# cbalint13/opencv-dlco

Hardware: AMD Instinct MI355X
Metric: pj-learn patch-pairs/sec (higher is better)
Workload: dtype f32; 1 GPU; pj-learn configs[1] Liberty-shaped, rank ~64: 500000 pair-rows x PR-dim 8192, batch 200+200 per GPU (global 200+200), mu=0.0025 gamma=0.5, fp32, rank 48 after 3893 steps; device= (gfx950:sramecc+:xnack-), burn_in_steps=300

## Files before the change

### include/dlco.h

```cpp
#ifndef DLCO_H
#define DLCO_H

#include <stddef.h>
#include <stdint.h>

#ifdef __cplusplus
extern "C" {
#endif

#define DLCO_OK            0
#define DLCO_ERR_INVALID  -2
#define DLCO_ERR_HIP      -3
#define DLCO_ERR_NODEVICE -4
#define DLCO_ERR_NOCONV   -5
#define DLCO_ERR_COMM     -6

typedef struct dlco_ctx dlco_ctx;

typedef struct dlco_cfg {
    int32_t  F;
    int32_t  N;
    int32_t  B;
    float    mu;
    float    gamma;
// ... 86 lines not shown
    int32_t        rows, ld;
    int32_t        kmajor;
    const int32_t *row_ids, *row_ids2;
    const float   *row_scale;
} dlco_gemm_operand;
typedef struct dlco_gemm_probe_args {
    int32_t M, N, K;
    dlco_gemm_operand A, B;
    const float *B2_host;
    int32_t split_k, k_dev, small_m_tiles, small_n_tiles, depth, reps;
    float   alpha, beta, b1, b2;
    const float *E1_host, *E2_host;
} dlco_gemm_probe_args;
int dlco_gemm_probe(dlco_ctx *ctx, const dlco_gemm_probe_args *args, float *C_host, float *C2_host, int32_t *depth_used,
                    double *us_per_launch);
int dlco_hinge_sum(dlco_ctx *ctx, const float *pos_host, int32_t n_pos,
                   const float *neg_host, int32_t n_neg, double *out);
int dlco_roc_stats(dlco_ctx *ctx, const float *dist_host, const uint8_t *labels_host, int32_t n,
                   float *fpr95, double *auc);

typedef struct dlco_log_entry {
    uint32_t t;
    int32_t  is_best;
    int32_t  saved;
    float    loss_val, regul, obj, obj_best;
    int32_t  rank, rank_best;
    int32_t  dim;
    double   auc, auc_best;
    float    fpr95, fpr95_best;
    double   vtime;
// ... 131 lines not shown
```

### opencv-dlco_amd/__init__.py

```python
import ctypes as C
import os
import subprocess

import numpy as np

_HERE = os.path.dirname(os.path.abspath(__file__))
LIB_PATH = os.path.join(_HERE, "libdlco.so")
HEADER_PATH = os.path.join(os.path.dirname(_HERE), "include", "dlco.h")

OK, ERR_INVALID, ERR_HIP, ERR_NODEVICE, ERR_NOCONV, ERR_COMM = 0, -2, -3, -4, -5, -6
BUF_DIST, BUF_GRAD, BUF_DFAVG, BUF_W, BUF_GATHER, BUF_DATA = 1, 2, 3, 4, 5, 6
ALLGATHER_FN = C.CFUNCTYPE(C.c_int, C.c_void_p, C.c_int32, C.c_size_t)
DETECT_THRESHOLD = 100 * 100 * 256 * 256


class DlcoError(RuntimeError):
    def __init__(self, code, msg):
        super().__init__("libdlco error %d: %s" % (code, msg))
        self.code = code


class Cfg(C.Structure):
    _fields_ = [
        ("F", C.c_int32), ("N", C.c_int32), ("B", C.c_int32),
# ... 22 lines not shown
    _fields_ = [
        ("host", C.POINTER(C.c_float)), ("rows", C.c_int32), ("ld", C.c_int32), ("kmajor", C.c_int32),
        ("row_ids", C.POINTER(C.c_int32)), ("row_ids2", C.POINTER(C.c_int32)), ("row_scale", C.POINTER(C.c_float)),
    ]


class GemmProbeArgs(C.Structure):
    _fields_ = [
        ("M", C.c_int32), ("N", C.c_int32), ("K", C.c_int32),
        ("A", GemmOperand), ("B", GemmOperand),
        ("B2_host", C.POINTER(C.c_float)),
        ("split_k", C.c_int32), ("k_dev", C.c_int32), ("small_m_tiles", C.c_int32), ("small_n_tiles", C.c_int32),
        ("depth", C.c_int32), ("reps", C.c_int32),
        ("alpha", C.c_float), ("beta", C.c_float), ("b1", C.c_float), ("b2", C.c_float),
        ("E1_host", C.POINTER(C.c_float)), ("E2_host", C.POINTER(C.c_float)),
    ]


def build(verbose=False):
    cmd = ["make", "-C", os.path.join(_HERE, "csrc"), "-j8"]
    if not verbose:
        cmd.insert(1, "-s")
    subprocess.check_call(cmd)


_lib = None
f32p, i32p, u8p = C.POINTER(C.c_float), C.POINTER(C.c_int32), C.POINTER(C.c_uint8)


def load():
# ... 34 lines not shown
    L.dlco_get_batch.argtypes = [vp, i32p, i32p, f32p, f32p, i32p, i32p]
    L.dlco_get_t.argtypes = [vp, C.POINTER(C.c_uint32)]
    L.dlco_get_W.argtypes = [vp, f32p, i32p]
    L.dlco_get_A.argtypes = [vp, f32p]
    L.dlco_get_dfavg.argtypes = [vp, f32p]
    L.dlco_set_state.argtypes = [vp, C.c_uint32, f32p, f32p, C.c_int32]
    L.dlco_validate.argtypes = [vp, f32p, f32p, i32p]
    L.dlco_stats.argtypes = [vp, f32p, C.c_int32, i32p, f32p, C.POINTER(C.c_double)]
    L.dlco_project_sqdist.argtypes = [vp, i32p, C.c_int32, f32p, C.c_int32, f32p]
    L.dlco_viol_counts.argtypes = [vp, f32p, f32p, C.c_int32, i32p, i32p]
    L.dlco_grad_rda.argtypes = [vp, i32p, i32p, i32p, i32p, C.c_int32, C.c_float, C.c_float, f32p, f32p]
    L.dlco_psd_project.argtypes = [vp, f32p, C.c_uint32, f32p, i32p, f32p]
    L.dlco_hinge_sum.argtypes = [vp, f32p, C.c_int32, f32p, C.c_int32, C.POINTER(C.c_double)]
    L.dlco_sym_product.argtypes = [vp, f32p, C.c_int32, f32p, C.c_int32, f32p]
    L.dlco_gemm_probe.argtypes = [vp, C.POINTER(GemmProbeArgs), f32p, f32p, i32p, C.POINTER(C.c_double)]
    L.dlco_roc_stats.argtypes = [vp, f32p, u8p, C.c_int32, f32p, C.POINTER(C.c_double)]
    L.dlco_log_step.argtypes = [vp, C.POINTER(LogEntry)]
    L.dlco_get_saved.argtypes = [vp, f32p, i32p, f32p]
    L.dlco_profile_enable.argtypes = [vp, C.c_int32]
    L.dlco_profile_read.argtypes = [vp, C.c_char_p, C.POINTER(C.c_int64), C.POINTER(C.c_double)]
    L.dlco_eig_stats.argtypes = [vp, C.POINTER(C.c_int64), C.POINTER(C.c_int64), C.POINTER(C.c_int64), i32p]
    L.dlco_counters.argtypes = [vp, C.POINTER(C.c_int64)]
    i64 = C.c_int64
    L.dlco_set_pairs_device.argtypes = [vp, vp, C.c_int32, i32p]
    L.dlco_desc_last_error.restype = C.c_char_p
    L.dlco_desc_last_error.argtypes = [vp]
    L.dlco_desc_create.argtypes = [C.POINTER(vp), C.c_float, C.c_int32, C.c_int32, C.c_int32]
    L.dlco_desc_destroy.argtypes = [vp]
    L.dlco_desc_destroy.restype = None
    L.dlco_desc_select_filters.argtypes = [f32p, C.c_int32, C.c_int32, f32p, C.c_int32, f32p, C.POINTER(C.c_int32)]
# ... 352 lines not shown
        twin = None if B2 is None else _f32(B2)
        assert twin is None or twin.shape == b.shape
        e1, e2 = (None if e is None else _f32(e) for e in (E1, E2))
        assert all(e is None or e.shape == (M, N) for e in (e1, e2))
        a.B2_host, a.E1_host, a.E2_host = _p(twin, f32p), _p(e1, f32p), _p(e2, f32p)
        a.split_k, a.k_dev, a.depth, a.reps = split_k, k_dev, depth, reps
        a.small_m_tiles, a.small_n_tiles = int(small_m_tiles), int(small_n_tiles)
        a.alpha, a.beta, a.b1, a.b2 = alpha, beta, b1, b2
        out = np.zeros((M, N), np.float32) if C_in is None else np.array(C_in, dtype=np.float32, order="C")
        assert out.shape == (M, N)
        out2 = None if twin is None else out.copy()
        used, us = C.c_int32(), C.c_double()
        self._ck(self.L.dlco_gemm_probe(self.h, C.byref(a), _p(out, f32p), _p(out2, f32p), C.byref(used), C.byref(us)))
        return dict(C=out, C2=out2, depth=used.value, us=us.value if reps else None)

    def hinge_sum(self, pos, neg):
        p, n = _f32(pos), _f32(neg)
        out = C.c_double()
        self._ck(self.L.dlco_hinge_sum(self.h, _p(p, f32p), p.size, _p(n, f32p), n.size, C.byref(out)))
        return out.value

    def roc_stats(self, dist, labels):
        d, l = _f32(dist), np.ascontiguousarray(labels, np.uint8).ravel()
        f, a = C.c_float(), C.c_double()
        self._ck(self.L.dlco_roc_stats(self.h, _p(d, f32p), _p(l, u8p), d.size, C.byref(f), C.byref(a)))
        return f.value, a.value

    def profile_enable(self, on=True):
        self._ck(self.L.dlco_profile_enable(self.h, int(on)))

# ... 485 lines not shown
```

### opencv-dlco_amd/csrc/dlco_api.cpp

```cpp
#include "../../include/dlco.h"

#include "dlco_internal.hpp"
#include "eig_tracker.hpp"
#include "pair_index.hpp"
#include "rccl_comm.hpp"
#include "host_comm.hpp"

#include <algorithm>
#include <cfloat>
#include <chrono>
#include <cmath>
#include <cstring>

using namespace dlco;

static thread_local std::string g_last_error;

namespace {
struct EnvSwitch { const char *name, *purpose; };
const EnvSwitch kEnvSwitches[] = {
    {"DLCO_SYRK_FP32", "gradient SYRK as the k-ordered fp32 MFMA chain (syrk_rda_kernel8) instead of split-bf16 planes"},
    {"DLCO_NO_PACKED", "full F x F dual average where the packed upper-tile form would apply"},
    {"DLCO_FORCE_SHARD", "column-sharded layout (cfg.shard) on a single rank: the multi-GPU path on one GPU"},
    {"DLCO_NO_RANK_UPDATE", "first filter term from a product with the dual average, not from the step's rank update"},
// ... 43 lines not shown
    int32_t *pin_ids = nullptr;
    uint32_t upload_ctr = 0;
    struct IdView { int32_t *p = nullptr; };
    DevBuf<int32_t> ids_all;
    IdView pos_rows, neg_rows, local_ids;
    const float *pd_cur = nullptr, *nd_cur = nullptr;
    DevBuf<int32_t> rho, kappa, act_ids, seed_ids, act_slot;
    bool rank_update = false;
    int planes_mode = 0;
    const float *ru_proj = nullptr;
    int ru_rows = 0;
    DevBuf<float> act_w, seed_w, dist_x, pd, nd, proj_slab, vproj, vdist, hrows;
    DevBuf<char> pplane[3];
    float *xdist = nullptr, *xgrad = nullptr;
    DevBuf<int> k_active;
    DevBuf<double> dscal;
    size_t proj_slab_floats = 0;
    int phase = 0;
    EigTracker *eig = nullptr;
    DevBuf<char> syrk_planes;
    RocWork *roc = nullptr;
    int64_t nonconv_steps = 0, steps_run = 0, active_rows_sum = 0;
    int32_t nonconv_window = 0;

    double auc_best = 0.0;
    float obj_best = FLT_MAX, fpr95_best = FLT_MAX;
    int r_best = 0;
    DevBuf<float> W_save_dev;
    int r_save = 0;
    int r_save_dev = 0;
// ... 145 lines not shown
    c->vproj.alloc((size_t)r * VCHUNK);
    for (int c0 = 0; c0 < n; c0 += VCHUNK) {
        const int nc = std::min(VCHUNK, n - c0);
        GemmArgs g;
        g.M = r; g.N = nc; g.K = c->F;
        g.A.p = Wd; g.A.ld = c->F; g.A.kmajor = false;
        g.B.ld = c->F; g.B.kmajor = false;
        if (rr.a) { g.B.p = c->dists; g.B.row_ids = rr.a + c0; g.B.row_ids2 = rr.b ? rr.b + c0 : nullptr; }
        else g.B.p = c->dists + (size_t)(row0 + c0) * c->F;
        g.C = c->vproj.p; g.ldc = VCHUNK;
        gemm_f32(g, c->stream);
        sqdist_from_proj(c->vproj.p, 1, r, nc, VCHUNK, out_dev + c0, c->stream);
    }
}

void project_few(dlco_ctx *c, const int32_t *ids_dev, int n, const float *Wd, int r, float *out_dev, int r_ext = 0)
{
    c->ru_proj = nullptr; c->ru_rows = 0;
    if (n <= 0) return;
    if (r <= 0) { fill_f32(out_dev, 0.f, (size_t)n, c->stream); return; }
    const int rp = std::max(r, r_ext);
    if (c->cfg.grad_bf16 && rp <= 96) {
        const int blocks = (n + 127) / 128;
        int ks = 1;
        while (ks * 2 * blocks <= 256 && (c->F / 64) % (ks * 2) == 0) ks *= 2;
        const size_t need = (size_t)(ks + 1) * rp * n;
        if (need > c->proj_slab_floats) { sync(c); c->proj_slab.alloc(need); c->proj_slab_floats = need; }
        float *reduced = rp > r ? c->proj_slab.p + (size_t)ks * rp * n : nullptr;
        for (auto &pl : c->pplane) pl.alloc(project_rows_plane_bytes(c->F));
        const RowRef rr = rows_of(c, ids_dev, 0, n);
        c->prof.begin(PROF_PROJECT);
// ... 19 lines not shown
    const int bn = (n <= 64 || bm == 64) ? 64 : 128;
    const long tiles = (long)((rp + bm - 1) / bm) * ((n + bn - 1) / bn);
    const int split = split_k_slices(tiles, 512, c->F, 128, LONG_MAX);
    const size_t need = (size_t)(split + 1) * rp * n;
    if (need > c->proj_slab_floats) { sync(c); c->proj_slab.alloc(need); c->proj_slab_floats = need; }
    float *proj = c->proj_slab.p + (size_t)split * rp * n;
    GemmArgs g;
    g.M = rp; g.N = n; g.K = c->F;
    g.A.p = Wd; g.A.ld = c->F; g.A.kmajor = false;
    const RowRef rr = rows_of(c, ids_dev, 0, n);
    g.B.p = c->dists; g.B.ld = c->F; g.B.kmajor = false; g.B.row_ids = rr.a; g.B.row_ids2 = rr.b;
    g.C = proj; g.ldc = n;
    g.split_k = split; g.slab = c->proj_slab.p;
    g.small_m_tiles = bm == 64;
    g.small_n_tiles = bn == 64;
    c->prof.begin(PROF_PROJECT);
    gemm_f32(g, c->stream);
    sqdist_from_proj(proj, 1, r, n, n, out_dev, c->stream);
    c->prof.end(PROF_PROJECT);
    if (rp > r) { c->ru_proj = proj; c->ru_rows = rp; }
}

void grad_syrk(dlco_ctx *c, const int32_t *ids, const float *w, const int *k_dev, int kmax, float alpha, float beta,
               float *dst, bool packed = false, const RankCoeffJob *coeff_job = nullptr)
{
    const int kpad = (kmax + 31) & ~31;
    const RowRef rr = rows_of(c, ids, 0, kpad);
    if (c->F % 128 == 0 && (reinterpret_cast<uintptr_t>(c->dists) & 15) == 0 &&
        (!c->shard || (c->comm.c0 % 128 == 0 && c->comm.cw % 128 == 0))) {
        c->prof.begin(PROF_GRAD_SYRK);
        const size_t pbytes = syrk_planes_bytes(kpad, c->F);
        if (pbytes > c->syrk_planes.n) { sync(c); c->syrk_planes.alloc(pbytes); }
        SyrkArgs a;
// ... 50 lines not shown
    const int B = c->B, Bl = c->Bl;
    for (int k = 0; k < B; k++) {
        const int ip = c->rng.uniform(0, c->idx.n_pos_trn);
        const int in = c->rng.uniform(0, c->idx.n_neg_trn);
        c->h_pos_rows[k] = c->idx.pos[ip];
        c->h_neg_rows[k] = c->idx.neg[in];
    }
    const size_t n_ids = (size_t)2 * B + 2 * Bl;
    int32_t *slot = c->pin_ids + (size_t)(c->upload_ctr++ & 1u) * n_ids;
    std::memcpy(slot, c->h_pos_rows.data(), B * sizeof(int32_t));
    std::memcpy(slot + B, c->h_neg_rows.data(), B * sizeof(int32_t));
    std::memcpy(slot + 2 * B, c->h_pos_rows.data() + c->lo, Bl * sizeof(int32_t));
    std::memcpy(slot + 2 * B + Bl, c->h_neg_rows.data() + c->lo, Bl * sizeof(int32_t));
    DLCO_HIP(hipMemcpyAsync(c->ids_all.p, slot, n_ids * sizeof(int32_t), hipMemcpyHostToDevice, c->stream));
    const int r_ext = (c->rank_update && c->r > 0 && c->eig->ext_rows() > c->r) ? c->eig->ext_rows() : 0;
    project_few(c, c->local_ids.p, 2 * Bl, c->W.p, c->r, c->xdist + (size_t)c->cfg.rank * 2 * Bl, r_ext);
    c->phase = 1;
}

void step_grad(dlco_ctx *c)
{
    DLCO_CHECK(c->phase == 1, DLCO_ERR_INVALID, "dlco_step_grad: call dlco_step_begin first");
    DLCO_CHECK(!c->shard, DLCO_ERR_INVALID, "dlco_step_grad: a sharded context steps with dlco_step");
    const int B = c->B, Bl = c->Bl, world = c->cfg.world;
    gather_dists(c, &c->pd_cur, &c->nd_cur);
    viol_counts_active_rows(c->pd_cur, c->nd_cur, B, c->rho.p, c->kappa.p, c->pos_rows.p, c->neg_rows.p, c->lo, c->lo + Bl,
                            c->act_ids.p, c->act_w.p, c->k_active.p, c->act_slot.p, c->stream);
    float alpha, beta;
    rda_coeffs(c, &alpha, &beta);
    RankCoeffJob job;
    const bool have_job = c->rank_update && c->planes_mode == 3 && c->ru_proj && world == 1 && c->eig->rank_coeff_job(&job, (2 * Bl + 31) & ~31);
    if (have_job) { job.proj = c->ru_proj; job.ldp = 2 * Bl; job.slot = c->act_slot.p; }
    if (world == 1) grad_syrk(c, c->act_ids.p, c->act_w.p, c->k_active.p, 2 * Bl, alpha, beta, c->dfavg.p, c->packed, have_job ? &job : nullptr);
    else grad_syrk(c, c->act_ids.p, c->act_w.p, c->k_active.p, 2 * Bl, 1.0f, 0.0f, c->xgrad);
    if (c->rank_update && c->ru_proj && c->syrk_planes.p) {
        RankUpdate ru;
        ru.proj = c->ru_proj; ru.ldp = 2 * Bl; ru.rows = c->ru_rows;
        ru.slot = c->act_slot.p; ru.w = c->act_w.p; ru.k_dev = c->k_active.p; ru.kmax = (2 * Bl + 31) & ~31;
        ru.planes = c->syrk_planes.p; ru.alpha = alpha; ru.beta = beta;
        ru.coeff_ready = have_job && job.m == c->ru_rows;
        ru.planes_mode = c->planes_mode;
        c->eig->offer_rank_update(ru);
// ... 156 lines not shown
        const int B = c->B;
        c->h_pos_rows.assign(B, 0); c->h_neg_rows.assign(B, 0);
        DLCO_HIP(hipHostMalloc((void **)&c->pin_ids, (size_t)2 * (2 * B + 2 * c->Bl) * sizeof(int32_t)));
        c->ids_all.alloc((size_t)2 * B + 2 * c->Bl);
        c->pos_rows.p = c->ids_all.p; c->neg_rows.p = c->ids_all.p + B; c->local_ids.p = c->ids_all.p + 2 * B;
        c->rho.alloc(B); c->kappa.alloc(B);
        const int kcap = (2 * B + 31) & ~31;
        c->act_ids.alloc(kcap); c->act_w.alloc(kcap); c->seed_ids.alloc(kcap); c->seed_w.alloc(kcap); c->act_slot.alloc(kcap);
        c->planes_mode = syrk_planes_mode(cfg->grad_bf16 != 0);
        c->rank_update = c->packed && cfg->world == 1 && c->planes_mode != 0 && env_switch("DLCO_NO_RANK_UPDATE") == nullptr;
        c->eig->set_emit_guards(c->rank_update);
        c->dist_x.alloc(2 * B); c->pd.alloc(B); c->nd.alloc(B);
        c->xdist = c->dist_x.p; c->xgrad = c->grad.p;
        c->k_active.alloc(4);
        c->k_active.zero(c->stream);
        c->eig->set_readback_extra(c->k_active.p);
        if (c->cfg.world == 1 || c->shard) {
            c->eig->set_growth_rows([c](float *dst, int want) -> int {
                if (c->phase != 2 || !c->have_data) return 0;
                const int k = c->eig->readback_extra();
                if (k <= 0 || k > 2 * c->B) return 0;
                const int cnt = std::min(want, k);
                if (cnt <= 0) return 0;
                const RowRef rr = rows_of(c, c->act_ids.p + (k - cnt), 0, cnt);
                scale_rows(dst, c->F, c->dists, c->F, nullptr, rr.a, rr.b, cnt, c->F, c->stream);
                return cnt;
            });
        }
        c->dscal.alloc(4);
        if (c->shard) {
// ... 648 lines not shown
            float ms = 0.f;
            DLCO_HIP(hipEventElapsedTime(&ms, e0, e1));
            (void)hipEventDestroy(e0); (void)hipEventDestroy(e1);
            if (us_per_launch) *us_per_launch = 1e3 * ms / a->reps;
        }
        h2d(c, C.p, C_host, mn * sizeof(float));
        if (C2_host) h2d(c, C2.p, C2_host, mn * sizeof(float));
        gemm_f32(g, c->stream);
        sync(c);
        d2h(c, C_host, C.p, mn * sizeof(float));
        if (C2_host) d2h(c, C2_host, C2.p, mn * sizeof(float));
        if (depth_used) *depth_used = used;
    });
}

int dlco_hinge_sum(dlco_ctx *c, const float *pos_host, int32_t n_pos, const float *neg_host, int32_t n_neg, double *out)
{
    if (!c || !out || n_pos < 0 || n_neg < 0) return DLCO_ERR_INVALID;
    return guarded(c, [&] {
        DLCO_HIP(hipSetDevice(c->cfg.device));
        *out = 0.0;
        if (n_pos == 0) return;
        DevBuf<float> p, n, rows;
        p.alloc(n_pos); n.alloc(std::max(n_neg, 1)); rows.alloc(n_pos);
        h2d(c, p.p, pos_host, (size_t)n_pos * sizeof(float));
        if (n_neg) h2d(c, n.p, neg_host, (size_t)n_neg * sizeof(float));
        hinge_rows(p.p, n_pos, n.p, n_neg, rows.p, c->stream);
        sum_f32_to_f64(rows.p, n_pos, c->dscal.p, c->stream);
        d2h(c, out, c->dscal.p, sizeof(double));
    });
// ... 128 lines not shown
```

### opencv-dlco_amd/csrc/dlco_internal.hpp

```cpp
#pragma once

#include "../../include/dlco.h"
#include "match_slices.hpp"

#include <hip/hip_runtime.h>

#include <algorithm>
#include <climits>
#include <cstdint>
#include <cstdio>
#include <cstdlib>
#include <cstring>
#include <functional>
#include <mutex>
#include <utility>
#include <stdexcept>
#include <string>
#include <type_traits>
#include <vector>

namespace patch_rules { struct Frame; }

namespace dlco {

// ... 134 lines not shown
};

struct GemmArgs {
    int M = 0, N = 0, K = 0;
    GemmOperand A, B;
    float *C = nullptr;
    long ldc = 0;
    float alpha = 1.0f, beta = 0.0f;
    const float *E1 = nullptr;
    float b1 = 0.0f;
    const float *E2 = nullptr;
    float b2 = 0.0f;
    const int *k_dev = nullptr;
    int split_k = 1;
    float *slab = nullptr;
    bool upper_only = false;
    const float *B2 = nullptr;
    float *C2 = nullptr;
    bool small_m_tiles = false;
    bool small_n_tiles = false;
    int depth = 0;
    int *depth_used = nullptr;
};

void gemm_f32(const GemmArgs &a, hipStream_t s);
int gemm_ring_depth();
size_t bf16x2_plane_bytes(int M, int K);
size_t bf16x2_slab_floats(int M, int N, int ksplit);
void split_planes_bf16(const float *X, long ldx, int M, int K, void *hi, void *lo, void *lo2, hipStream_t s);
struct SplitPlanes {
    void *hi = nullptr, *lo = nullptr, *lo2 = nullptr;
};
struct SkinnyArgs {
    const float *X = nullptr;
    long ldx = 0;
    int M = 0;
    const float *G = nullptr;
    long ldg = 0;
    int N = 0, K = 0;
    float alpha = 1.0f;
// ... 85 lines not shown
    SplitPlanes out_planes;
};
bool rank_first_term(const RankTermBlock &b, const RankUpdate &ru, hipStream_t s);
size_t syrk_packed_floats(int F);
void syrk_pack_upper(const float *C, long ldc, int F, float *packed, hipStream_t s);
void syrk_unpack_upper(const float *packed, int F, float *C, long ldc, hipStream_t s);
bool skinny_product_sym(const SkinnyArgs &a, hipStream_t s);
size_t gemm_slab_floats(int M, int N, int split_k);
inline int split_k_slices(long tiles, long target, long K, long kmin, long slab_cap)
{
    const long split = std::min(std::min((target + tiles - 1) / tiles, K / kmin), slab_cap);
    return (int)std::max(1L, split);
}
void splitk_reduce_f32(const float *slab, int split, int M, int N, float *C, long ldc, float alpha, float beta,
                       const float *E1, float b1, const float *E2, float b2, hipStream_t s);

void sqdist_from_proj(const float *proj, int split, int r, int n, long ld, float *dist, hipStream_t s, int r_all = 0,
                      float *reduced = nullptr);
void viol_counts(const float *pd, const float *nd, int B, int32_t *rho, int32_t *kappa, hipStream_t s);
void viol_counts_active_rows(const float *pd, const float *nd, int B, int32_t *rho, int32_t *kappa, const int32_t *pos_rows,
                             const int32_t *neg_rows, int slot_lo, int slot_hi, int32_t *ids, float *w, int *k_active, int32_t *slots,
                             hipStream_t s);
void build_active_rows(const int32_t *pos_rows, const int32_t *neg_rows, const int32_t *rho, const int32_t *kappa,
                       int B, int slot_lo, int slot_hi, int32_t *ids, float *w, int *k_active, hipStream_t s);
void hinge_rows(const float *pos, int n_pos, const float *neg, int n_neg, float *row_sums, hipStream_t s);
void sum_f32_to_f64(const float *x, int n, double *out, hipStream_t s);
void hinge_rows_batched(const float *pos, int n_pos, const float *neg, int n_neg, long ld_in, float *row_sums, long ld_out, int count,
                        hipStream_t s);
void sum_f32_to_f64_batched(const float *x, int n, long ldx, double *out, int count, hipStream_t s);
void axpby_inplace(float *y, const float *x, float a, float b, size_t n, hipStream_t s);
void scale_rows(float *dst, long ldd, const float *src, long lds, const float *scale, const int32_t *src_rows,
                const int32_t *src_rows2, int rows, int cols, hipStream_t s);
void emit_w_rows(float *W, long ldw, const float *Q, long ldq, const float *theta, int nw, float mu, float cscale, int F,
                 int m_ext, float *wscale, hipStream_t s);
void translate_ids(const int32_t *ids, int base, int n, const int32_t *pa, const int32_t *pb, int32_t *out_a, int32_t *out_b,
                   hipStream_t s);
void fill_f32(float *p, float v, size_t n, hipStream_t s);
// ... 101 lines not shown
```

### opencv-dlco_amd/csrc/kernels_gemm.hip

```cpp
#include "dlco_internal.hpp"

namespace dlco {

typedef float f32x16 __attribute__((ext_vector_type(16)));
typedef float f32x4 __attribute__((ext_vector_type(4)));

namespace {

constexpr int BK = 16;
constexpr int PAD = 4;
constexpr int NT = 256;
#ifndef DLCO_GEMM_DEPTH
#define DLCO_GEMM_DEPTH 4
#endif
constexpr int RING_DEPTH = DLCO_GEMM_DEPTH;
static_assert(RING_DEPTH == 2 || RING_DEPTH == 4 || RING_DEPTH == 8, "ring depth: 2, 4 or 8");

struct OperandDev {
    const float *p;
    long ld;
    const int32_t *row_ids;
    const float *row_scale;
    int vec_ok;
    const int32_t *row_ids2;
// ... 322 lines not shown
    else launch<WM, WN, 1>(g, akm, bkm, grid, s);
}

inline int vec_ok(const GemmOperand &o) { return (o.ld % 4 == 0) && ((reinterpret_cast<uintptr_t>(o.p) & 15) == 0); }

inline bool plain_operand(const GemmOperand &o, int t, int K)
{
    if (!vec_ok(o) || o.row_ids2 || (o.kmajor && (o.row_scale || o.row_ids))) return false;
    return (o.kmajor ? t : K) % 4 == 0;
}

}

size_t gemm_slab_floats(int M, int N, int split_k) { return split_k > 1 ? (size_t)split_k * M * N : 0; }

void splitk_reduce_f32(const float *slab, int split, int M, int N, float *C, long ldc, float alpha, float beta,
                       const float *E1, float b1, const float *E2, float b2, hipStream_t s)
{
    const long total = (long)M * N;
    auto al16 = [](const void *p) { return (reinterpret_cast<uintptr_t>(p) & 15) == 0; };
    if (split <= 32 && total >= 65536 && N % 4 == 0 && ldc % 4 == 0 && al16(slab) && al16(C) && (!E1 || al16(E1)) &&
        (!E2 || al16(E2))) {
        long blocks = (total / 4 + 255) / 256;
        if (blocks > 4096) blocks = 4096;
        hipLaunchKernelGGL(splitk_reduce_wide_kernel, dim3((unsigned)blocks), dim3(256), 0, s, slab, split, M, N, C, ldc, alpha,
                           beta, E1, b1, E2, b2);
        DLCO_HIP(hipGetLastError());
        return;
    }
    long blocks = (total * 16 + 255) / 256;
    if (blocks > 8192) blocks = 8192;
    hipLaunchKernelGGL(splitk_reduce_kernel, dim3((unsigned)blocks), dim3(256), 0, s, slab, split, M, N, C, ldc, alpha, beta,
                       E1, b1, E2, b2);
    DLCO_HIP(hipGetLastError());
}

int gemm_ring_depth() { return RING_DEPTH; }

void gemm_f32(const GemmArgs &a, hipStream_t s)
{
    if (a.M <= 0 || a.N <= 0) return;
    DLCO_CHECK(a.depth == 0 || a.depth == 1, -2, "gemm_f32: depth is 0 (the library's choice) or 1");
    DLCO_CHECK(a.A.p && a.B.p && a.C, -2, "gemm_f32: null operand");
    DLCO_CHECK(!(a.upper_only && (a.M != a.N || a.split_k > 1)), -2, "gemm_f32: upper_only needs M==N, split_k==1");
    GemmDev g;
    g.M = a.M; g.N = a.N; g.K = a.K;
    g.A = {a.A.p, a.A.ld, a.A.row_ids, a.A.kmajor ? a.A.row_scale : nullptr, vec_ok(a.A), a.A.row_ids2};
    g.B = {a.B.p, a.B.ld, a.B.row_ids, a.B.kmajor ? a.B.row_scale : nullptr, vec_ok(a.B), a.B.row_ids2};
    g.C = a.C; g.ldc = a.ldc;
    g.alpha = a.alpha; g.beta = a.beta; g.E1 = a.E1; g.b1 = a.b1; g.E2 = a.E2; g.b2 = a.b2;
    g.k_dev = a.k_dev;
    g.upper_only = a.upper_only ? 1 : 0;
    int split = a.split_k < 1 ? 1 : a.split_k;
    int chunk = (a.K + split - 1) / split;
    chunk = ((chunk + BK - 1) / BK) * BK;
    if (chunk < BK) chunk = BK;
    split = a.K > 0 ? (a.K + chunk - 1) / chunk : 1;
    g.k_chunk = chunk;
    g.slab = nullptr;
    if (split > 1) {
        DLCO_CHECK(a.slab != nullptr, -2, "gemm_f32: split_k > 1 needs a slab workspace");
        g.slab = a.slab;
    }
    g.B2 = a.B2; g.C2 = a.C2;
    if (a.B2) {
        DLCO_CHECK(a.C2 && split == 1 && !a.upper_only, -2, "gemm_f32: a twin product needs C2 and no K split");
        split = 2;
    }
    bool small_m = a.M <= 64 || a.small_m_tiles, small_n = a.N <= 64 || a.small_n_tiles;
    auto n_wg = [&](bool sm, bool sn) {
        return (long)((a.M + (sm ? 63 : 127)) / (sm ? 64 : 128)) * ((a.N + (sn ? 63 : 127)) / (sn ? 64 : 128)) * split;
    };
    if (!a.upper_only) {
// ... 4 lines not shown
    if (a.depth_used) *a.depth_used = ring && (small_m || small_n) ? RING_DEPTH : 1;
    if (small_m && small_n) {
        dim3 grid((a.N + 63) / 64, (a.M + 63) / 64, split);
        launch_small<1, 1>(g, a.A.kmajor, a.B.kmajor, grid, ring, s);
    } else if (small_m) {
        dim3 grid((a.N + 127) / 128, (a.M + 63) / 64, split);
        launch_small<1, 2>(g, a.A.kmajor, a.B.kmajor, grid, ring, s);
    } else if (small_n) {
        dim3 grid((a.N + 63) / 64, (a.M + 127) / 128, split);
        launch_small<2, 1>(g, a.A.kmajor, a.B.kmajor, grid, ring, s);
    } else {
        dim3 grid((a.N + 127) / 128, (a.M + 127) / 128, split);
        launch<2, 2, 1>(g, a.A.kmajor, a.B.kmajor, grid, s);
    }
    DLCO_HIP(hipGetLastError());
    if (split > 1 && !a.B2)
        splitk_reduce_f32(a.slab, split, a.M, a.N, a.C, a.ldc, a.alpha, a.beta, a.E1, a.b1, a.E2, a.b2, s);
}

}
```

### opencv-dlco_amd/csrc/kernels_step.hip

```cpp
#include "dlco_internal.hpp"

#include <algorithm>

namespace dlco {

namespace {

__device__ __forceinline__ double wave_sum_d(double v)
{
#pragma unroll
    for (int o = 32; o > 0; o >>= 1) v += __shfl_xor(v, o, 64);
    return v;
}

__global__ void sqdist_kernel(const float *proj, int split, int r, int n, long ld, float *dist)
{
    const int j = blockIdx.x * blockDim.x + threadIdx.x;
    if (j >= n) return;
    const long plane = (long)r * ld;
    float d = 0.f;
    int q = 0;
    if (split == 1) {
        for (; q + 8 <= r; q += 8) {
            float v[8];
#pragma unroll
            for (int u = 0; u < 8; u++) v[u] = proj[(long)(q + u) * ld + j];
#pragma unroll
            for (int u = 0; u < 8; u++) d += v[u] * v[u];
        }
    }
    for (; q < r; q++) {
        float p = 0.f;
        for (int z = 0; z < split; z++) p += proj[z * plane + (long)q * ld + j];
        d += p * p;
    }
    dist[j] = d;
}

__global__ __launch_bounds__(512) void sqdist_split_kernel(const float *proj, int split, int r, int n, long ld, float *dist, int r_all,
                                                           float *reduced)
{
    __shared__ float p[96][64];
    const int jl = threadIdx.x & 63, qg = threadIdx.x >> 6;
    const int j = blockIdx.x * 64 + jl;
    const long plane = (long)r_all * ld;
    float d = 0.f;
    for (int q0 = 0; q0 < r_all; q0 += 96) {
        const int qn = min(96, r_all - q0);
        for (int q = qg; q < qn; q += 8) {
// ... 9 lines not shown
                    for (int u = 0; u < 8; u++) acc += v[u];
                }
                for (; z < split; z++) acc += src[z * plane];
            }
            p[q][jl] = acc;
            if (reduced && j < n) reduced[(long)(q0 + q) * ld + j] = acc;
        }
        __syncthreads();
        if (qg == 0)
            for (int q = 0; q < min(qn, r - q0); q++) d += p[q][jl] * p[q][jl];
        __syncthreads();
    }
    if (qg == 0 && j < n) dist[j] = d;
}

__device__ __forceinline__ void viol_body(float *sh, const float *pd, const float *nd, int B, int32_t *rho, int32_t *kappa)
{
    float *spd = sh, *snd = sh + B;
    for (int i = threadIdx.x; i < B; i += blockDim.x) { spd[i] = pd[i] + 1.0f; snd[i] = nd[i]; }
    __syncthreads();
    for (int i = threadIdx.x; i < B; i += blockDim.x) {
        const float thr = spd[i];
        int c = 0;
        for (int j = 0; j < B; j++) c += (thr > snd[j]) ? 1 : 0;
        rho[i] = c;
        const float me = snd[i];
        int k = 0;
        for (int j = 0; j < B; j++) k += (spd[j] > me) ? 1 : 0;
        kappa[i] = k;
    }
}
__global__ void viol_kernel(const float *pd, const float *nd, int B, int32_t *rho, int32_t *kappa)
{
    extern __shared__ float sh[];
    viol_body(sh, pd, nd, B, rho, kappa);
}

__device__ __forceinline__ void active_rows_body(const int32_t *pos_rows, const int32_t *neg_rows, const int32_t *rho,
                                                 const int32_t *kappa, int B, int lo, int hi, int32_t *ids, float *w, int *k_active,
                                                 int32_t *slots = nullptr)
{
    __shared__ int wave_cnt[16];
    __shared__ int base;
    const int tid = threadIdx.x, lane = tid & 63, wave = tid >> 6, nw = blockDim.x >> 6;
    const int n_own = max(0, min(hi, B) - lo), total = 2 * n_own;
    if (tid == 0) base = 0;
// ... 27 lines not shown
    for (int z = k + tid; z < ((2 * B + 31) & ~31); z += blockDim.x) { ids[z] = 0; w[z] = 0.f; }
}
__global__ void active_rows_kernel(const int32_t *pos_rows, const int32_t *neg_rows, const int32_t *rho,
                                   const int32_t *kappa, int B, int lo, int hi, int32_t *ids, float *w, int *k_active)
{
    active_rows_body(pos_rows, neg_rows, rho, kappa, B, lo, hi, ids, w, k_active);
}
__global__ void viol_active_kernel(const float *pd, const float *nd, int B, int32_t *rho, int32_t *kappa, const int32_t *pos_rows,
                                   const int32_t *neg_rows, int lo, int hi, int32_t *ids, float *w, int *k_active, int32_t *slots)
{
    extern __shared__ float sh[];
    viol_body(sh, pd, nd, B, rho, kappa);
    __threadfence_block();
    __syncthreads();
    active_rows_body(pos_rows, neg_rows, rho, kappa, B, lo, hi, ids, w, k_active, slots);
}

__global__ __launch_bounds__(256) void hinge_rows_kernel(const float *pos, int n_pos, const float *neg, int n_neg,
                                                         float *row_sums, long ld_in, long ld_out)
{
    __shared__ float sn[2048];
    pos += blockIdx.y * ld_in;
    neg += blockIdx.y * ld_in;
    row_sums += blockIdx.y * ld_out;
    const int i = blockIdx.x * blockDim.x + threadIdx.x;
    const float base = (i < n_pos) ? pos[i] + 1.0f : 0.f;
    float tsum = 0.f;
    for (int j0 = 0; j0 < n_neg; j0 += 2048) {
        const int cnt = min(2048, n_neg - j0);
        __syncthreads();
// ... 148 lines not shown
    hipLaunchKernelGGL(viol_kernel, dim3(1), dim3(256), 2 * B * sizeof(float), s, pd, nd, B, rho, kappa);
    DLCO_HIP(hipGetLastError());
}

void viol_counts_active_rows(const float *pd, const float *nd, int B, int32_t *rho, int32_t *kappa, const int32_t *pos_rows,
                             const int32_t *neg_rows, int slot_lo, int slot_hi, int32_t *ids, float *w, int *k_active, int32_t *slots,
                             hipStream_t s)
{
    if (B <= 0) return;
    DLCO_CHECK(B <= 8192, -2, "viol_counts: batch too large for one workgroup's LDS");
    hipLaunchKernelGGL(viol_active_kernel, dim3(1), dim3(256), 2 * B * sizeof(float), s, pd, nd, B, rho, kappa, pos_rows, neg_rows, slot_lo,
                       slot_hi, ids, w, k_active, slots);
    DLCO_HIP(hipGetLastError());
}

void build_active_rows(const int32_t *pos_rows, const int32_t *neg_rows, const int32_t *rho, const int32_t *kappa,
                       int B, int slot_lo, int slot_hi, int32_t *ids, float *w, int *k_active, hipStream_t s)
{
    hipLaunchKernelGGL(active_rows_kernel, dim3(1), dim3(256), 0, s, pos_rows, neg_rows, rho, kappa, B, slot_lo, slot_hi,
                       ids, w, k_active);
    DLCO_HIP(hipGetLastError());
}

void hinge_rows(const float *pos, int n_pos, const float *neg, int n_neg, float *row_sums, hipStream_t s)
{
    if (n_pos <= 0) return;
    hipLaunchKernelGGL(hinge_rows_kernel, dim3((n_pos + 255) / 256), dim3(256), 0, s, pos, n_pos, neg, n_neg, row_sums, 0L, 0L);
    DLCO_HIP(hipGetLastError());
}

// ... 91 lines not shown
```

Before: 736,200 pair-rows/s.

## Fuse split-K reduce, sqdist and violation counting into one step-head kernel

Adds a step_head kernel that sums the GEMM's split-K slabs, and uses a last-block ticket so one workgroup then computes squared distances, violation counts and active rows. For single-device unsharded runs with small batches it replaces three launches (split-K reduce, sqdist, viol_active), and the later viol_counts call is skipped when the head already ran. This cuts launch overhead and intermediate round trips on the per-step critical path. In exchange, the tail work is serialized on a single workgroup, relies on an atomic ticket and cross-block visibility, and adds a probe API for checking the fused path against the unfused one.

New measurement: 740,800 pair-rows/s (median of 6 runs). No clear change (+0.6%).

```diff
diff --git a/include/dlco.h b/include/dlco.h
--- a/include/dlco.h
+++ b/include/dlco.h
@@ -124,6 +124,14 @@
 } dlco_gemm_probe_args;
 int dlco_gemm_probe(dlco_ctx *ctx, const dlco_gemm_probe_args *args, float *C_host, float *C2_host, int32_t *depth_used,
                     double *us_per_launch);
+typedef struct dlco_step_head_probe_args {
+    const float   *slab_host;
+    int32_t        split, r_all, r, B;
+    const int32_t *pos_rows, *neg_rows;
+    int32_t        fused;
+} dlco_step_head_probe_args;
+int dlco_step_head_probe(dlco_ctx *ctx, const dlco_step_head_probe_args *args, float *proj, float *dist, int32_t *rho,
+                         int32_t *kappa, int32_t *ids, float *w, int32_t *k_active, int32_t *slots);
 int dlco_hinge_sum(dlco_ctx *ctx, const float *pos_host, int32_t n_pos,
                    const float *neg_host, int32_t n_neg, double *out);
 int dlco_roc_stats(dlco_ctx *ctx, const float *dist_host, const uint8_t *labels_host, int32_t n,
diff --git a/opencv-dlco_amd/__init__.py b/opencv-dlco_amd/__init__.py
--- a/opencv-dlco_amd/__init__.py
+++ b/opencv-dlco_amd/__init__.py
@@ -60,6 +60,15 @@
         ("depth", C.c_int32), ("reps", C.c_int32),
         ("alpha", C.c_float), ("beta", C.c_float), ("b1", C.c_float), ("b2", C.c_float),
         ("E1_host", C.POINTER(C.c_float)), ("E2_host", C.POINTER(C.c_float)),
+    ]
+
+
+class StepHeadProbeArgs(C.Structure):
+    _fields_ = [
+        ("slab_host", C.POINTER(C.c_float)),
+        ("split", C.c_int32), ("r_all", C.c_int32), ("r", C.c_int32), ("B", C.c_int32),
+        ("pos_rows", C.POINTER(C.c_int32)), ("neg_rows", C.POINTER(C.c_int32)),
+        ("fused", C.c_int32),
     ]
 
 
@@ -124,6 +133,7 @@
     L.dlco_hinge_sum.argtypes = [vp, f32p, C.c_int32, f32p, C.c_int32, C.POINTER(C.c_double)]
     L.dlco_sym_product.argtypes = [vp, f32p, C.c_int32, f32p, C.c_int32, f32p]
     L.dlco_gemm_probe.argtypes = [vp, C.POINTER(GemmProbeArgs), f32p, f32p, i32p, C.POINTER(C.c_double)]
+    L.dlco_step_head_probe.argtypes = [vp, C.POINTER(StepHeadProbeArgs), f32p, f32p, i32p, i32p, i32p, f32p, i32p, i32p]
     L.dlco_roc_stats.argtypes = [vp, f32p, u8p, C.c_int32, f32p, C.POINTER(C.c_double)]
     L.dlco_log_step.argtypes = [vp, C.POINTER(LogEntry)]
     L.dlco_get_saved.argtypes = [vp, f32p, i32p, f32p]
@@ -506,6 +516,21 @@
         self._ck(self.L.dlco_gemm_probe(self.h, C.byref(a), _p(out, f32p), _p(out2, f32p), C.byref(used), C.byref(us)))
         return dict(C=out, C2=out2, depth=used.value, us=us.value if reps else None)
 
+    def step_head_probe(self, slabs, r, pos_rows, neg_rows, fused=True):
+        s = _f32(slabs)
+        assert s.ndim == 3 and s.shape[2] % 2 == 0
+        split, r_all, n = s.shape
+        B, kcap = n // 2, (n + 31) & ~31
+        pr, nr = _i32(pos_rows), _i32(neg_rows)
+        assert pr.size == B and nr.size == B
+        a = StepHeadProbeArgs(_p(s, f32p), split, r_all, r, B, _p(pr, i32p), _p(nr, i32p), int(fused))
+        proj, dist, w = np.empty((r_all, n), np.float32), np.empty(n, np.float32), np.empty(kcap, np.float32)
+        rho, kappa, ids, slots = (np.empty(k, np.int32) for k in (B, B, kcap, kcap))
+        k = C.c_int32()
+        self._ck(self.L.dlco_step_head_probe(self.h, C.byref(a), _p(proj, f32p), _p(dist, f32p), _p(rho, i32p), _p(kappa, i32p),
+                                             _p(ids, i32p), _p(w, f32p), C.byref(k), _p(slots, i32p)))
+        return dict(proj=proj, dist=dist, rho=rho, kappa=kappa, ids=ids, w=w, k_active=k.value, slots=slots)
+
     def hinge_sum(self, pos, neg):
         p, n = _f32(pos), _f32(neg)
         out = C.c_double()
diff --git a/opencv-dlco_amd/csrc/dlco_api.cpp b/opencv-dlco_amd/csrc/dlco_api.cpp
--- a/opencv-dlco_amd/csrc/dlco_api.cpp
+++ b/opencv-dlco_amd/csrc/dlco_api.cpp
@@ -81,6 +81,8 @@
     DevBuf<char> pplane[3];
     float *xdist = nullptr, *xgrad = nullptr;
     DevBuf<int> k_active;
+    DevBuf<unsigned> head_ticket;
+    bool counts_made = false;
     DevBuf<double> dscal;
     size_t proj_slab_floats = 0;
     int phase = 0;
@@ -256,7 +258,8 @@
     }
 }
 
-void project_few(dlco_ctx *c, const int32_t *ids_dev, int n, const float *Wd, int r, float *out_dev, int r_ext = 0)
+void project_few(dlco_ctx *c, const int32_t *ids_dev, int n, const float *Wd, int r, float *out_dev, int r_ext = 0,
+                 StepHeadArgs *head = nullptr)
 {
     c->ru_proj = nullptr; c->ru_rows = 0;
     if (n <= 0) return;
@@ -306,9 +309,18 @@
     g.split_k = split; g.slab = c->proj_slab.p;
     g.small_m_tiles = bm == 64;
     g.small_n_tiles = bn == 64;
+    const int slices = gemm_k_slices(g.K, split);
+    const bool fused = head && n == 2 * head->B && head->B <= STEP_HEAD_MAX_B &&
+                       (slices == 1 || splitk_reduce_butterfly(g.slab, slices, rp, n, proj, n, nullptr, nullptr));
+    g.keep_slabs = fused;
     c->prof.begin(PROF_PROJECT);
     gemm_f32(g, c->stream);
-    sqdist_from_proj(proj, 1, r, n, n, out_dev, c->stream);
+    if (fused) {
+        head->slab = g.slab; head->split = slices; head->r_all = rp; head->r = r;
+        head->proj = proj; head->dist = out_dev;
+        step_head(*head, c->stream);
+        c->counts_made = true;
+    } else sqdist_from_proj(proj, 1, r, n, n, out_dev, c->stream);
     c->prof.end(PROF_PROJECT);
     if (rp > r) { c->ru_proj = proj; c->ru_rows = rp; }
 }
@@ -389,7 +401,14 @@
     std::memcpy(slot + 2 * B + Bl, c->h_neg_rows.data() + c->lo, Bl * sizeof(int32_t));
     DLCO_HIP(hipMemcpyAsync(c->ids_all.p, slot, n_ids * sizeof(int32_t), hipMemcpyHostToDevice, c->stream));
     const int r_ext = (c->rank_update && c->r > 0 && c->eig->ext_rows() > c->r) ? c->eig->ext_rows() : 0;
-    project_few(c, c->local_ids.p, 2 * Bl, c->W.p, c->r, c->xdist + (size_t)c->cfg.rank * 2 * Bl, r_ext);
+    StepHeadArgs head;
+    head.B = B; head.ticket = c->head_ticket.p;
+    head.rho = c->rho.p; head.kappa = c->kappa.p; head.pos_rows = c->pos_rows.p; head.neg_rows = c->neg_rows.p;
+    head.lo = c->lo; head.hi = c->lo + Bl;
+    head.ids = c->act_ids.p; head.w = c->act_w.p; head.k_active = c->k_active.p; head.slots = c->act_slot.p;
+    c->counts_made = false;
+    project_few(c, c->local_ids.p, 2 * Bl, c->W.p, c->r, c->xdist + (size_t)c->cfg.rank * 2 * Bl, r_ext,
+                c->cfg.world == 1 && !c->shard ? &head : nullptr);
     c->phase = 1;
 }
 
@@ -399,8 +418,9 @@
     DLCO_CHECK(!c->shard, DLCO_ERR_INVALID, "dlco_step_grad: a sharded context steps with dlco_step");
     const int B = c->B, Bl = c->Bl, world = c->cfg.world;
     gather_dists(c, &c->pd_cur, &c->nd_cur);
-    viol_counts_active_rows(c->pd_cur, c->nd_cur, B, c->rho.p, c->kappa.p, c->pos_rows.p, c->neg_rows.p, c->lo, c->lo + Bl,
-                            c->act_ids.p, c->act_w.p, c->k_active.p, c->act_slot.p, c->stream);
+    if (!c->counts_made)
+        viol_counts_active_rows(c->pd_cur, c->nd_cur, B, c->rho.p, c->kappa.p, c->pos_rows.p, c->neg_rows.p, c->lo, c->lo + Bl,
+                                c->act_ids.p, c->act_w.p, c->k_active.p, c->act_slot.p, c->stream);
     float alpha, beta;
     rda_coeffs(c, &alpha, &beta);
     RankCoeffJob job;
@@ -587,6 +607,8 @@
         c->xdist = c->dist_x.p; c->xgrad = c->grad.p;
         c->k_active.alloc(4);
         c->k_active.zero(c->stream);
+        c->head_ticket.alloc(1);
+        c->head_ticket.zero(c->stream);
         c->eig->set_readback_extra(c->k_active.p);
         if (c->cfg.world == 1 || c->shard) {
             c->eig->set_growth_rows([c](float *dst, int want) -> int {
@@ -1265,6 +1287,58 @@
     });
 }
 
+int dlco_step_head_probe(dlco_ctx *c, const dlco_step_head_probe_args *a, float *proj_host, float *dist_host, int32_t *rho_host,
+                         int32_t *kappa_host, int32_t *ids_host, float *w_host, int32_t *k_active_host, int32_t *slots_host)
+{
+    if (!c || !a || !a->slab_host || !a->pos_rows || !a->neg_rows || !proj_host || !dist_host || !rho_host || !kappa_host || !ids_host ||
+        !w_host || !k_active_host || !slots_host)
+        return DLCO_ERR_INVALID;
+    if (a->split < 1 || a->r < 1 || a->r_all < a->r || a->B < 1 || a->B > STEP_HEAD_MAX_B) return DLCO_ERR_INVALID;
+    return guarded(c, [&] {
+        DLCO_HIP(hipSetDevice(c->cfg.device));
+        DLCO_CHECK(c->phase == 0, DLCO_ERR_INVALID, "dlco_step_head_probe: step in flight");
+        const int B = a->B, n = 2 * B, kcap = (n + 31) & ~31;
+        const size_t mn = (size_t)a->r_all * n;
+        DevBuf<float> slab, proj, dist, w;
+        DevBuf<int32_t> rows, rho, kappa, ids, slots;
+        DevBuf<int> k;
+        slab.alloc((size_t)a->split * mn); proj.alloc(mn); dist.alloc(n); w.alloc(kcap);
+        rows.alloc(n); rho.alloc(B); kappa.alloc(B); ids.alloc(kcap); slots.alloc(kcap); k.alloc(1);
+        DLCO_CHECK(a->split == 1 || splitk_reduce_butterfly(slab.p, a->split, a->r_all, n, proj.p, n, nullptr, nullptr), DLCO_ERR_INVALID,
+                   "dlco_step_head_probe: the library sums this shape's slices by its wide form");
+        h2d(c, slab.p, a->slab_host, (size_t)a->split * mn * sizeof(float));
+        h2d(c, rows.p, a->pos_rows, (size_t)B * sizeof(int32_t));
+        h2d(c, rows.p + B, a->neg_rows, (size_t)B * sizeof(int32_t));
+        DLCO_HIP(hipMemsetAsync(proj.p, 0xFF, mn * sizeof(float), c->stream));
+        DLCO_HIP(hipMemsetAsync(dist.p, 0xFF, (size_t)n * sizeof(float), c->stream));
+        DLCO_HIP(hipMemsetAsync(w.p, 0xFF, (size_t)kcap * sizeof(float), c->stream));
+        for (DevBuf<int32_t> *b : {&rho, &kappa}) DLCO_HIP(hipMemsetAsync(b->p, 0xFF, (size_t)B * sizeof(int32_t), c->stream));
+        for (DevBuf<int32_t> *b : {&ids, &slots}) DLCO_HIP(hipMemsetAsync(b->p, 0xFF, (size_t)kcap * sizeof(int32_t), c->stream));
+        DLCO_HIP(hipMemsetAsync(k.p, 0xFF, sizeof(int), c->stream));
+        if (a->split == 1) DLCO_HIP(hipMemcpyAsync(proj.p, slab.p, mn * sizeof(float), hipMemcpyDeviceToDevice, c->stream));
+        if (a->fused) {
+            StepHeadArgs h;
+            h.slab = slab.p; h.split = a->split; h.r_all = a->r_all; h.r = a->r; h.B = B;
+            h.proj = proj.p; h.dist = dist.p; h.ticket = c->head_ticket.p;
+            h.rho = rho.p; h.kappa = kappa.p; h.pos_rows = rows.p; h.neg_rows = rows.p + B; h.lo = 0; h.hi = B;
+            h.ids = ids.p; h.w = w.p; h.k_active = k.p; h.slots = slots.p;
+            step_head(h, c->stream);
+        } else {
+            if (a->split > 1) splitk_reduce_f32(slab.p, a->split, a->r_all, n, proj.p, n, 1.0f, 0.0f, nullptr, 0.f, nullptr, 0.f, c->stream);
+            sqdist_from_proj(proj.p, 1, a->r, n, n, dist.p, c->stream);
+            viol_counts_active_rows(dist.p, dist.p + B, B, rho.p, kappa.p, rows.p, rows.p + B, 0, B, ids.p, w.p, k.p, slots.p, c->stream);
+        }
+        d2h(c, proj_host, proj.p, mn * sizeof(float));
+        d2h(c, dist_host, dist.p, (size_t)n * sizeof(float));
+        d2h(c, rho_host, rho.p, (size_t)B * sizeof(int32_t));
+        d2h(c, kappa_host, kappa.p, (size_t)B * sizeof(int32_t));
+        d2h(c, ids_host, ids.p, (size_t)kcap * sizeof(int32_t));
+        d2h(c, w_host, w.p, (size_t)kcap * sizeof(float));
+        d2h(c, k_active_host, k.p, sizeof(int));
+        d2h(c, slots_host, slots.p, (size_t)kcap * sizeof(int32_t));
+    });
+}
+
 int dlco_hinge_sum(dlco_ctx *c, const float *pos_host, int32_t n_pos, const float *neg_host, int32_t n_neg, double *out)
 {
     if (!c || !out || n_pos < 0 || n_neg < 0) return DLCO_ERR_INVALID;
diff --git a/opencv-dlco_amd/csrc/dlco_internal.hpp b/opencv-dlco_amd/csrc/dlco_internal.hpp
--- a/opencv-dlco_amd/csrc/dlco_internal.hpp
+++ b/opencv-dlco_amd/csrc/dlco_internal.hpp
@@ -172,6 +172,7 @@
     const int *k_dev = nullptr;
     int split_k = 1;
     float *slab = nullptr;
+    bool keep_slabs = false;
     bool upper_only = false;
     const float *B2 = nullptr;
     float *C2 = nullptr;
@@ -182,6 +183,7 @@
 };
 
 void gemm_f32(const GemmArgs &a, hipStream_t s);
+int gemm_k_slices(int K, int split_k);
 int gemm_ring_depth();
 size_t bf16x2_plane_bytes(int M, int K);
 size_t bf16x2_slab_floats(int M, int N, int ksplit);
@@ -297,6 +299,7 @@
 }
 void splitk_reduce_f32(const float *slab, int split, int M, int N, float *C, long ldc, float alpha, float beta,
                        const float *E1, float b1, const float *E2, float b2, hipStream_t s);
+bool splitk_reduce_butterfly(const float *slab, int split, int M, int N, const float *C, long ldc, const float *E1, const float *E2);
 
 void sqdist_from_proj(const float *proj, int split, int r, int n, long ld, float *dist, hipStream_t s, int r_all = 0,
                       float *reduced = nullptr);
@@ -304,6 +307,21 @@
 void viol_counts_active_rows(const float *pd, const float *nd, int B, int32_t *rho, int32_t *kappa, const int32_t *pos_rows,
                              const int32_t *neg_rows, int slot_lo, int slot_hi, int32_t *ids, float *w, int *k_active, int32_t *slots,
                              hipStream_t s);
+constexpr int STEP_HEAD_MAX_B = 2048;
+struct StepHeadArgs {
+    const float *slab = nullptr;
+    int split = 1, r_all = 0, r = 0, B = 0;
+    float *proj = nullptr, *dist = nullptr;
+    unsigned *ticket = nullptr;
+    int32_t *rho = nullptr, *kappa = nullptr;
+    const int32_t *pos_rows = nullptr, *neg_rows = nullptr;
+    int lo = 0, hi = 0;
+    int32_t *ids = nullptr;
+    float *w = nullptr;
+    int *k_active = nullptr;
+    int32_t *slots = nullptr;
+};
+void step_head(const StepHeadArgs &a, hipStream_t s);
 void build_active_rows(const int32_t *pos_rows, const int32_t *neg_rows, const int32_t *rho, const int32_t *kappa,
                        int B, int slot_lo, int slot_hi, int32_t *ids, float *w, int *k_active, hipStream_t s);
 void hinge_rows(const float *pos, int n_pos, const float *neg, int n_neg, float *row_sums, hipStream_t s);
diff --git a/opencv-dlco_amd/csrc/kernels_gemm.hip b/opencv-dlco_amd/csrc/kernels_gemm.hip
--- a/opencv-dlco_amd/csrc/kernels_gemm.hip
+++ b/opencv-dlco_amd/csrc/kernels_gemm.hip
@@ -360,13 +360,27 @@
 
 size_t gemm_slab_floats(int M, int N, int split_k) { return split_k > 1 ? (size_t)split_k * M * N : 0; }
 
+static int slice_chunk(int K, int split_k)
+{
+    const int split = split_k < 1 ? 1 : split_k;
+    int chunk = (K + split - 1) / split;
+    chunk = ((chunk + BK - 1) / BK) * BK;
+    return chunk < BK ? BK : chunk;
+}
+int gemm_k_slices(int K, int split_k) { return K > 0 ? (K + slice_chunk(K, split_k) - 1) / slice_chunk(K, split_k) : 1; }
+
+bool splitk_reduce_butterfly(const float *slab, int split, int M, int N, const float *C, long ldc, const float *E1, const float *E2)
+{
+    auto al16 = [](const void *p) { return (reinterpret_cast<uintptr_t>(p) & 15) == 0; };
+    return !(split <= 32 && (long)M * N >= 65536 && N % 4 == 0 && ldc % 4 == 0 && al16(slab) && al16(C) && (!E1 || al16(E1)) &&
+             (!E2 || al16(E2)));
+}
+
 void splitk_reduce_f32(const float *slab, int split, int M, int N, float *C, long ldc, float alpha, float beta,
                        const float *E1, float b1, const float *E2, float b2, hipStream_t s)
 {
     const long total = (long)M * N;
-    auto al16 = [](const void *p) { return (reinterpret_cast<uintptr_t>(p) & 15) == 0; };
-    if (split <= 32 && total >= 65536 && N % 4 == 0 && ldc % 4 == 0 && al16(slab) && al16(C) && (!E1 || al16(E1)) &&
-        (!E2 || al16(E2))) {
+    if (!splitk_reduce_butterfly(slab, split, M, N, C, ldc, E1, E2)) {
         long blocks = (total / 4 + 255) / 256;
         if (blocks > 4096) blocks = 4096;
         hipLaunchKernelGGL(splitk_reduce_wide_kernel, dim3((unsigned)blocks), dim3(256), 0, s, slab, split, M, N, C, ldc, alpha,
@@ -397,12 +411,8 @@
     g.alpha = a.alpha; g.beta = a.beta; g.E1 = a.E1; g.b1 = a.b1; g.E2 = a.E2; g.b2 = a.b2;
     g.k_dev = a.k_dev;
     g.upper_only = a.upper_only ? 1 : 0;
-    int split = a.split_k < 1 ? 1 : a.split_k;
-    int chunk = (a.K + split - 1) / split;
-    chunk = ((chunk + BK - 1) / BK) * BK;
-    if (chunk < BK) chunk = BK;
-    split = a.K > 0 ? (a.K + chunk - 1) / chunk : 1;
-    g.k_chunk = chunk;
+    int split = gemm_k_slices(a.K, a.split_k);
+    g.k_chunk = slice_chunk(a.K, a.split_k);
     g.slab = nullptr;
     if (split > 1) {
         DLCO_CHECK(a.slab != nullptr, -2, "gemm_f32: split_k > 1 needs a slab workspace");
@@ -437,7 +447,7 @@
         launch<2, 2, 1>(g, a.A.kmajor, a.B.kmajor, grid, s);
     }
     DLCO_HIP(hipGetLastError());
-    if (split > 1 && !a.B2)
+    if (split > 1 && !a.B2 && !a.keep_slabs)
         splitk_reduce_f32(a.slab, split, a.M, a.N, a.C, a.ldc, a.alpha, a.beta, a.E1, a.b1, a.E2, a.b2, s);
 }
 
diff --git a/opencv-dlco_amd/csrc/kernels_step.hip b/opencv-dlco_amd/csrc/kernels_step.hip
--- a/opencv-dlco_amd/csrc/kernels_step.hip
+++ b/opencv-dlco_amd/csrc/kernels_step.hip
@@ -12,6 +12,15 @@
     for (int o = 32; o > 0; o >>= 1) v += __shfl_xor(v, o, 64);
     return v;
 }
+
+__device__ __forceinline__ float sq_add8(float d, const float *v)
+{
+#pragma clang fp contract(off)
+#pragma unroll
+    for (int u = 0; u < 8; u++) { const float t = v[u] * v[u]; d = d + t; }
+    return d;
+}
+__device__ __forceinline__ float sq_add_tail(float d, float v) { return __builtin_fmaf(v, v, d); }
 
 __global__ void sqdist_kernel(const float *proj, int split, int r, int n, long ld, float *dist)
 {
@@ -25,14 +34,13 @@
             float v[8];
 #pragma unroll
             for (int u = 0; u < 8; u++) v[u] = proj[(long)(q + u) * ld + j];
-#pragma unroll
-            for (int u = 0; u < 8; u++) d += v[u] * v[u];
+            d = sq_add8(d, v);
         }
     }
     for (; q < r; q++) {
         float p = 0.f;
         for (int z = 0; z < split; z++) p += proj[z * plane + (long)q * ld + j];
-        d += p * p;
+        d = sq_add_tail(d, p);
     }
     dist[j] = d;
 }
@@ -72,11 +80,8 @@
     if (qg == 0 && j < n) dist[j] = d;
 }
 
-__device__ __forceinline__ void viol_body(float *sh, const float *pd, const float *nd, int B, int32_t *rho, int32_t *kappa)
-{
-    float *spd = sh, *snd = sh + B;
-    for (int i = threadIdx.x; i < B; i += blockDim.x) { spd[i] = pd[i] + 1.0f; snd[i] = nd[i]; }
-    __syncthreads();
+__device__ __forceinline__ void viol_count_body(const float *spd, const float *snd, int B, int32_t *rho, int32_t *kappa)
+{
     for (int i = threadIdx.x; i < B; i += blockDim.x) {
         const float thr = spd[i];
         int c = 0;
@@ -88,6 +93,13 @@
         kappa[i] = k;
     }
 }
+__device__ __forceinline__ void viol_body(float *sh, const float *pd, const float *nd, int B, int32_t *rho, int32_t *kappa)
+{
+    float *spd = sh, *snd = sh + B;
+    for (int i = threadIdx.x; i < B; i += blockDim.x) { spd[i] = pd[i] + 1.0f; snd[i] = nd[i]; }
+    __syncthreads();
+    viol_count_body(spd, snd, B, rho, kappa);
+}
 __global__ void viol_kernel(const float *pd, const float *nd, int B, int32_t *rho, int32_t *kappa)
 {
     extern __shared__ float sh[];
@@ -145,6 +157,77 @@
     __threadfence_block();
     __syncthreads();
     active_rows_body(pos_rows, neg_rows, rho, kappa, B, lo, hi, ids, w, k_active, slots);
+}
+
+constexpr int HEAD_T = 512, HEAD_ZT = 3, HEAD_QB = 64;
+__global__ __launch_bounds__(HEAD_T) void step_head_kernel(StepHeadArgs a)
+{
+    extern __shared__ float sh[];
+    __shared__ int last;
+    const int tid = threadIdx.x, n = 2 * a.B;
+    const long total = (long)a.r_all * n;
+    if (a.split > 1) {
+        const long e = (long)blockIdx.x * HEAD_T + tid;
+        if (e < total) {
+            float s[16];
+#pragma unroll
+            for (int z = 0; z < 16; z++) s[z] = 0.f;
+            for (int z0 = 0; z0 < a.split; z0 += 16 * HEAD_ZT) {
+                float v[HEAD_ZT][16];
+#pragma unroll
+                for (int t = 0; t < HEAD_ZT; t++)
+#pragma unroll
+                    for (int z = 0; z < 16; z++) v[t][z] = a.slab[(long)min(z0 + 16 * t + z, a.split - 1) * total + e];
+#pragma unroll
+                for (int t = 0; t < HEAD_ZT; t++)
+#pragma unroll
+                    for (int z = 0; z < 16; z++)
+                        if (z0 + 16 * t + z < a.split) s[z] += v[t][z];
+            }
+#pragma unroll
+            for (int w = 1; w < 16; w <<= 1)
+#pragma unroll
+                for (int z = 0; z < 16; z += 2 * w) s[z] += s[z + w];
+            __hip_atomic_store(a.proj + e, s[0], __ATOMIC_RELAXED, __HIP_MEMORY_SCOPE_AGENT);
+        }
+        asm volatile("s_waitcnt vmcnt(0)" ::: "memory");
+    }
+    __syncthreads();
+    if (tid == 0) {
+        const unsigned t = __hip_atomic_fetch_add(a.ticket, 1u, __ATOMIC_RELAXED, __HIP_MEMORY_SCOPE_AGENT);
+        last = t == gridDim.x - 1 ? 1 : 0;
+        if (last) __hip_atomic_store(a.ticket, 0u, __ATOMIC_RELAXED, __HIP_MEMORY_SCOPE_AGENT);
+    }
+    __syncthreads();
+    if (!last) return;
+    __builtin_amdgcn_fence(__ATOMIC_ACQUIRE, "wavefront");
+    for (int j = tid; j < n; j += HEAD_T) {
+        const float *src = a.proj + j;
+        float d = 0.f;
+        int q = 0;
+        for (; q + HEAD_QB <= a.r; q += HEAD_QB) {
+            float v[HEAD_QB];
+#pragma unroll
+            for (int u = 0; u < HEAD_QB; u++) v[u] = __hip_atomic_load(src + (long)(q + u) * n, __ATOMIC_RELAXED, __HIP_MEMORY_SCOPE_AGENT);
+#pragma unroll
+            for (int u = 0; u < HEAD_QB; u += 8) d = sq_add8(d, v + u);
+        }
+        for (; q + 8 <= a.r; q += 8) {
+            float v[8];
+#pragma unroll
+            for (int u = 0; u < 8; u++) v[u] = __hip_atomic_load(src + (long)(q + u) * n, __ATOMIC_RELAXED, __HIP_MEMORY_SCOPE_AGENT);
+            d = sq_add8(d, v);
+        }
+        for (; q < a.r; q++) d = sq_add_tail(d, __hip_atomic_load(src + (long)q * n, __ATOMIC_RELAXED, __HIP_MEMORY_SCOPE_AGENT));
+        a.dist[j] = d;
+        sh[j] = j < a.B ? d + 1.0f : d;
+    }
+    __syncthreads();
+    int32_t *srho = reinterpret_cast<int32_t *>(sh + n), *skappa = srho + a.B;
+    viol_count_body(sh, sh + a.B, a.B, srho, skappa);
+    __syncthreads();
+    for (int i = tid; i < a.B; i += HEAD_T) { a.rho[i] = srho[i]; a.kappa[i] = skappa[i]; }
+    active_rows_body(a.pos_rows, a.neg_rows, srho, skappa, a.B, a.lo, a.hi, a.ids, a.w, a.k_active, a.slots);
 }
 
 __global__ __launch_bounds__(256) void hinge_rows_kernel(const float *pos, int n_pos, const float *neg, int n_neg,
@@ -323,6 +406,15 @@
     DLCO_HIP(hipGetLastError());
 }
 
+void step_head(const StepHeadArgs &a, hipStream_t s)
+{
+    DLCO_CHECK(a.B >= 1 && a.B <= STEP_HEAD_MAX_B && a.r >= 1 && a.r_all >= a.r && a.split >= 1, -2, "step_head: shape out of range");
+    DLCO_CHECK(a.split == 1 || a.slab, -2, "step_head: K slices without their slabs");
+    const long blocks = a.split > 1 ? ((long)a.r_all * 2 * a.B + HEAD_T - 1) / HEAD_T : 1;
+    hipLaunchKernelGGL(step_head_kernel, dim3((unsigned)blocks), dim3(HEAD_T), 4 * a.B * sizeof(float), s, a);
+    DLCO_HIP(hipGetLastError());
+}
+
 void build_active_rows(const int32_t *pos_rows, const int32_t *neg_rows, const int32_t *rho, const int32_t *kappa,
                        int B, int slot_lo, int slot_hi, int32_t *ids, float *w, int *k_active, hipStream_t s)
 {
```
